# niessner/BundleFusion

Measured on AMD Instinct MI355X. Metric: frames/sec end-to-end (SIFT+SBA+TSDF re-integrate), 640x480 @4mm, higher is better.
Workload: dtype f32

## Files before the change

### bundlefusion_amd/csrc/solver.hip

```cpp
#include <hip/hip_runtime.h>

#include <algorithm>
#include <cstring>
#include <vector>

#include "bf_device.h"
#include "bf_resources.h"
#include "bf_se3.h"

using namespace bf;

namespace {

constexpr float FLOAT_EPSILON = 0.000001f;
constexpr uint32_t NOSLOT = 0xFFFFFFFFu;
constexpr int DENSE_BLK = 120;

typedef float f32x4 __attribute__((ext_vector_type(4)));

enum Flag { FL_DONE = 0, FL_NUM_SLOTS = 1, FL_NUM_PAIRS = 2, FL_LIST_LEN = 3, FL_GN_ITERS = 4, FL_BARRIER_FAIL = 5, FL_SLOT_OVERFLOW = 6, FL_PCG_ITERS = 8, FL_COUNT = 40 };

struct Cfg {
    float denseDistThresh, denseNormalThresh, denseColorThresh, denseColorGradientMin, denseDepthMin, denseDepthMax;
    uint32_t subsample;
    uint32_t W, H;
    float fx, fy, cx, cy;
    float wSparse, wDepth, wColor;
    int usePairwise;
};

struct Dev {
    const bf_entry_j* corr; uint32_t C;
    const int* valid; uint32_t N;
    float* xRot; float* xTrans;
    m44* T; m44* Tinv;
    uint32_t *keyCount, *keyStart, *cursor, *slotOfKey, *denseRaw, *keyPair;
    uint32_t *rowStart, *slotCol, *slotKey, *corrList;
    float *slotD, *slotO, *slotG, *slotP;
    float *diagA, *rhs, *prec;
    float *delta, *r, *p, *Ap;
    uint2* densePairs; float* denseWeight; float* denseBlocks;
    const bf_cached_frame* cache;
    int* flags;
    int* gridBar;
    float* energies;
    float* maxRes; int* maxIdx; int* highCount;
    int* numEntriesPerRow;
    float* coopVec;
    uint32_t* scanRow;
    float* maxResPart; int* maxIdxPart;
    uint32_t maxSlots, maxPairs;
};

BF_DEV f3 ld3(const float* p) { return mk3(p[0], p[1], p[2]); }
BF_DEV bool validCorr(const bf_entry_j& c) { return c.imgIdx_i != 0xFFFFFFFFu; }

__global__ void k_solve_begin(Dev d) {
    for (uint32_t k = threadIdx.x; k < (uint32_t)FL_COUNT; k += blockDim.x) d.flags[k] = 0;
    for (uint32_t k = threadIdx.x; k < 32u; k += blockDim.x) d.gridBar[k] = 0;
}

__global__ void k_poses(Dev d, uint32_t numKeys, int useDense) {
    const uint32_t i = blockIdx.x * blockDim.x + threadIdx.x;
    for (uint32_t k = i; k < numKeys; k += gridDim.x * blockDim.x) {
        d.keyCount[k] = 0u; d.cursor[k] = 0u;
        if (useDense) { d.denseRaw[k] = 0u; d.keyPair[k] = 0u; }
    }
    if (d.flags[FL_DONE]) return;
    if (i >= d.N) return;
    const m44 M = poseToMatrix(ld3(d.xRot + 3 * i), ld3(d.xTrans + 3 * i));
    d.T[i] = M;
    d.Tinv[i] = inverse44(M);
}

__global__ void k_key_count(Dev d) {
    if (d.flags[FL_DONE]) return;
    const uint32_t c = blockIdx.x * blockDim.x + threadIdx.x;
    if (c >= d.C) return;
    const bf_entry_j e = d.corr[c];
    if (!validCorr(e) || e.imgIdx_i >= d.N || e.imgIdx_j >= d.N) return;
    atomicAdd(&d.keyCount[e.imgIdx_i * d.N + e.imgIdx_j], 1u);
    atomicAdd(&d.keyCount[e.imgIdx_j * d.N + e.imgIdx_i], 1u);
}

__global__ void k_row_entries(Dev d) {
    const uint32_t i = blockIdx.x * blockDim.x + threadIdx.x;
    if (i >= d.N) return;
    uint32_t n = 0;
    for (uint32_t j = 0; j < d.N; ++j) n += d.keyCount[i * d.N + j];
    d.numEntriesPerRow[i] = (int)n;
}

BF_DEV void scanKey(const Dev& d, int useDense, uint32_t N, uint32_t i, uint32_t j, uint32_t& cnt, uint32_t& dn) {
    cnt = d.keyCount[i * N + j];
    dn = (useDense && i != j) ? d.denseRaw[min(i, j) * N + max(i, j)] : 0u;
}

__global__ __launch_bounds__(64) void k_scan_rows(Dev d, int useDense) {
    if (d.flags[FL_DONE]) return;
    const uint32_t N = d.N, i = blockIdx.x, lane = threadIdx.x;
    uint32_t a = 0, b = 0, c = 0;
    for (uint32_t j = lane; j < N; j += 64) {
        uint32_t cnt, dn;
        scanKey(d, useDense, N, i, j, cnt, dn);
        a += cnt; b += (cnt > 0 || dn) ? 1u : 0u; c += (dn && i < j) ? 1u : 0u;
    }
    a = (uint32_t)wave_sum_i((int)a); b = (uint32_t)wave_sum_i((int)b); c = (uint32_t)wave_sum_i((int)c);
    if (lane == 0) { d.scanRow[i * 3 + 0] = a; d.scanRow[i * 3 + 1] = b; d.scanRow[i * 3 + 2] = c; }
}

__global__ __launch_bounds__(1024) void k_scan_base(Dev d) {
    if (d.flags[FL_DONE]) return;
    __shared__ uint32_t sA[1024], sB[1024], sC[1024];
    const uint32_t N = d.N;
    const uint32_t chunk = (N + blockDim.x - 1) / blockDim.x;
    const uint32_t r0 = min(threadIdx.x * chunk, N), r1 = min(r0 + chunk, N);
    uint32_t a = 0, b = 0, c = 0;
    for (uint32_t r = r0; r < r1; ++r) { a += d.scanRow[r * 3]; b += d.scanRow[r * 3 + 1]; c += d.scanRow[r * 3 + 2]; }
    sA[threadIdx.x] = a; sB[threadIdx.x] = b; sC[threadIdx.x] = c;
    __syncthreads();
    for (uint32_t off = 1; off < blockDim.x; off <<= 1) {
        uint32_t ta = 0, tb = 0, tc = 0;
        if (threadIdx.x >= off) { ta = sA[threadIdx.x - off]; tb = sB[threadIdx.x - off]; tc = sC[threadIdx.x - off]; }
        __syncthreads();
// ... 266 lines not shown
                        if (tx >= 0 && ty >= 0 && tx < (int)c.W && ty < (int)c.H) {
                            float ci[4], ni[4];
                            bilinear<4>(u, v, tgt.d_cameraposDownsampled, c.W, c.H, ci);
                            if (ci[2] > c.denseDepthMin && ci[2] < c.denseDepthMax) {
                                bilinear<4>(u, v, tgt.d_normalsDownsampled, c.W, c.H, ni);
                                if (ni[0] != BF_MINF) {
                                    const f3 ct = mk3(ci[0], ci[1], ci[2]);
                                    const f3 nt = mk3(ni[0], ni[1], ni[2]);
                                    const float dist = len3(cst - ct);
                                    const float dN = n4[0] * ni[0] + n4[1] * ni[1] + n4[2] * ni[2] + n4[3] * ni[3];
                                    if (dN >= c.denseNormalThresh && dist <= c.denseDistThresh) {
                                        float jI[3][6], jJ[3][6];
                                        if (i > 0) derivI(TjI, Ti, cs, jI);
                                        if (j > 0) derivJ(TiI, Tj, cs, jJ);
                                        if (useDepth) {
                                            const f3 diff = ct - cst;
                                            Xd[12] = dot3(diff, nt);
                                            wd = c.wDepth * pw * powf(fmaxf(0.0f, 1.0f - ct.z / 2.0f), 2.5f);
#pragma unroll
                                            for (int k = 0; k < 6; ++k) {
                                                if (i > 0) Xd[k] = -(jI[0][k] * nt.x + jI[1][k] * nt.y + jI[2][k] * nt.z);
                                                if (j > 0) Xd[6 + k] = -(jJ[0][k] * nt.x + jJ[1][k] * nt.y + jJ[2][k] * nt.z);
                                            }
                                        }
                                        if (useColor) {
                                            float dI[2], iT;
                                            bilinear<2>(u, v, tgt.d_intensityDerivsDownsampled, c.W, c.H, dI);
                                            bilinear<1>(u, v, tgt.d_intensityDownsampled, c.W, c.H, &iT);
                                            const float res = iT - src.d_intensityDownsampled[idx];
                                            if (dI[0] != BF_MINF && fabsf(res) < c.denseColorThresh &&
                                                sqrtf(dI[0] * dI[0] + dI[1] * dI[1]) > c.denseColorGradientMin) {
                                                const float z2 = cst.z * cst.z;
                                                const float P00 = c.fx / cst.z, P02 = -c.fx * cst.x / z2, P11 = c.fy / cst.z, P12 = -c.fy * cst.y / z2;
                                                Xc[12] = res;
                                                wc = c.wColor * pw * fmaxf(0.0f, 1.0f - fabsf(res) / (1.15f * c.denseColorThresh));
#pragma unroll
                                                for (int k = 0; k < 6; ++k) {
                                                    if (i > 0) Xc[k] = dI[0] * (P00 * jI[0][k] + 0.0f * jI[1][k] + P02 * jI[2][k]) + dI[1] * (0.0f * jI[0][k] + P11 * jI[1][k] + P12 * jI[2][k]);
                                                    if (j > 0) Xc[6 + k] = dI[0] * (P00 * jJ[0][k] + 0.0f * jJ[1][k] + P02 * jJ[2][k]) + dI[1] * (0.0f * jJ[0][k] + P11 * jJ[1][k] + P12 * jJ[2][k]);
                                                }
                                            }
                                        }
                                    }
                                }
                            }
                        }
                    }
                }
            }
#pragma unroll
            for (int pass = 0; pass < 2; ++pass) {
                if (pass == 0 && !useDepth) continue;
                if (pass == 1 && !useColor) continue;
#pragma unroll
                for (int k = 0; k < 13; ++k) tileX[wave][lane][k] = pass == 0 ? Xd[k] : Xc[k];
                tileX[wave][lane][13] = 0.0f; tileX[wave][lane][14] = 0.0f; tileX[wave][lane][15] = 0.0f;
                tileW[wave][lane] = pass == 0 ? wd : wc;
                __syncthreads();
#pragma unroll
                for (int g = 0; g < 16; g += 2) {
                    const int r0 = 4 * g + (int)(lane >> 4), r1 = r0 + 4;
                    const float b0 = tileX[wave][r0][lane & 15], b1 = tileX[wave][r1][lane & 15];
                    acc0 = __builtin_amdgcn_mfma_f32_16x16x4f32(tileW[wave][r0] * b0, b0, acc0, 0, 0, 0);
                    acc1 = __builtin_amdgcn_mfma_f32_16x16x4f32(tileW[wave][r1] * b1, b1, acc1, 0, 0, 0);
                }
                __syncthreads();
            }
        }
#pragma unroll
        for (int r = 0; r < 4; ++r) part[wave][(4 * (lane >> 4) + r) * 16 + (lane & 15)] = acc0[r] + acc1[r];
        __syncthreads();
        if (threadIdx.x < DENSE_BLK) {
            const uint32_t t = threadIdx.x;
            uint32_t row, col;
            if (t < 36) { row = t / 6; col = t % 6; }
            else if (t < 72) { row = 6 + (t - 36) / 6; col = 6 + (t - 36) % 6; }
            else if (t < 108) { row = (t - 72) / 6; col = 6 + (t - 72) % 6; }
            else if (t < 114) { row = t - 108; col = 12; }
            else { row = 6 + (t - 114); col = 12; }
            const uint32_t e = row * 16 + col;
            out[t] = ((part[0][e] + part[1][e]) + part[2][e]) + part[3][e];
        }
        __syncthreads();
    }
}

__global__ __launch_bounds__(256) void k_slots(Dev d, Cfg c, int useDense) {
    if (d.flags[FL_DONE]) return;
    const uint32_t nSlots = (uint32_t)d.flags[FL_NUM_SLOTS];
    const uint32_t lane = threadIdx.x & 63;
    const uint32_t wavesPerGrid = gridDim.x * (blockDim.x >> 6);
    for (uint32_t s = blockIdx.x * (blockDim.x >> 6) + (threadIdx.x >> 6); s < nSlots; s += wavesPerGrid) {
        const uint32_t key = d.slotKey[s];
        const uint32_t start = d.keyStart[key], cnt = d.keyCount[key];
        const uint32_t a = lane / 6, b = lane % 6;
        float accD = 0.0f, accO = 0.0f;
        uint32_t prev = 0;
        bool first = true;
        for (uint32_t k = 0; k < cnt; ++k) {
            uint32_t best = 0xFFFFFFFFu;
            for (uint32_t t = lane; t < cnt; t += 64) {
                const uint32_t v = d.corrList[start + t];
                if ((first || v > prev) && v < best) best = v;
            }
#pragma unroll
            for (int o = 32; o > 0; o >>= 1) { const uint32_t t = __shfl_xor(best, o, 64); best = t < best ? t : best; }
            prev = best; first = false;
            const bf_entry_j e = d.corr[best >> 1];
            const bool roleB = best & 1u;
            const m44 TI = d.T[e.imgIdx_i], TJ = d.T[e.imgIdx_j];
            const f3 wi = xform(TI, mk3(e.pos_i[0], e.pos_i[1], e.pos_i[2]));
            const f3 wj = xform(TJ, mk3(e.pos_j[0], e.pos_j[1], e.pos_j[2]));
            const f3 r = wi - wj;
            const f3 wx = roleB ? wj : wi, wy = roleB ? wi : wj;
            const float sx = roleB ? -1.0f : 1.0f;
            auto col = [](f3 w, uint32_t q) -> f3 {
                switch (q) {
                    case 0: return mk3(1.0f, 0.0f, 0.0f);
                    case 1: return mk3(0.0f, 1.0f, 0.0f);
                    case 2: return mk3(0.0f, 0.0f, 1.0f);
                    case 3: return mk3(0.0f, -w.z, w.y);
                    case 4: return mk3(w.z, 0.0f, -w.x);
                    default: return mk3(-w.y, w.x, 0.0f);
                }
            };
            if (lane < 36) {
                const f3 ja = col(wx, a);
                accD += dot3(ja, col(wx, b));
                accO += -dot3(ja, col(wy, b));
            } else if (lane < 42) {
                accD += sx * dot3(col(wx, lane - 36), r);
            } else if (lane < 45) {
                const f3 jq = col(wx, lane - 42 + 3);
                accD += dot3(jq, jq);
            } else if (lane == 45) {
                accD += 1.0f;
            }
        }
        float dD = 0.0f, dO = 0.0f;
        if (useDense) {
            const uint32_t pp = d.keyPair[key];
            if (pp) {
                const float* blk = d.denseBlocks + (size_t)(pp - 1) * DENSE_BLK;
                const uint32_t i = key / d.N, j = key % d.N;
                const bool fwd = i < j;
                if (lane < 36) {
                    dD = fwd ? blk[a * 6 + b] : blk[36 + a * 6 + b];
                    dO = fwd ? blk[72 + a * 6 + b] : blk[72 + b * 6 + a];
                } else if (lane < 42) {
                    dD = fwd ? blk[108 + (lane - 36)] : blk[114 + (lane - 36)];
                }
            }
        }
        if (lane < 36) {
            d.slotD[(size_t)s * 36 + lane] = c.wSparse * accD + dD;
            d.slotO[(size_t)s * 36 + lane] = c.wSparse * accO + dO;
        } else if (lane < 42) {
            d.slotG[(size_t)s * 6 + (lane - 36)] = c.wSparse * accD + dD;
        } else if (lane < 46) {
            d.slotP[(size_t)s * 4 + (lane - 42)] = accD;
        }
    }
}

__global__ __launch_bounds__(256) void k_rows(Dev d) {
    if (d.flags[FL_DONE]) return;
// ... 498 lines not shown
}

__global__ __launch_bounds__(64) void k_max_residual_final(Dev d, uint32_t G) {
    float best = 0.0f; int bi = 0;
    if (threadIdx.x < G) { best = d.maxResPart[threadIdx.x]; bi = d.maxIdxPart[threadIdx.x]; }
#pragma unroll
    for (int o = 32; o > 0; o >>= 1) {
        const float ov = __shfl_xor(best, o, 64); const int oi = __shfl_xor(bi, o, 64);
        if (maxResBetter(ov, oi, best, bi)) { best = ov; bi = oi; }
    }
    if (threadIdx.x == 0) { d.maxRes[0] = best; d.maxIdx[0] = bi; }
}

__global__ void k_count_high(Dev d, float w, float thresh) {
    const uint32_t c = blockIdx.x * blockDim.x + threadIdx.x;
    bool hi = false;
    if (c < d.C) hi = absMaxResidual(d, d.corr[c], w) > thresh;
    const unsigned long long m = __ballot(hi);
    if ((threadIdx.x & 63) == 0 && m) atomicAdd(d.highCount, __popcll(m));
}

__global__ __launch_bounds__(1024) void k_energy(Dev d, float w, uint32_t slot, int honourDone) {
    if (honourDone && d.flags[FL_DONE] && slot > (uint32_t)d.flags[FL_GN_ITERS]) return;
    __shared__ float sh[16];
    float part = 0.0f;
    for (uint32_t c = threadIdx.x; c < d.C; c += blockDim.x) {
        const bf_entry_j e = d.corr[c];
        if (!validCorr(e)) continue;
        const m44 TI = poseToMatrix(ld3(d.xRot + 3 * e.imgIdx_i), ld3(d.xTrans + 3 * e.imgIdx_i));
        const m44 TJ = poseToMatrix(ld3(d.xRot + 3 * e.imgIdx_j), ld3(d.xTrans + 3 * e.imgIdx_j));
        const f3 r = xform(TI, mk3(e.pos_i[0], e.pos_i[1], e.pos_i[2])) - xform(TJ, mk3(e.pos_j[0], e.pos_j[1], e.pos_j[2]));
        part += w * dot3(r, r);
    }
    const float tot = blockSum(part, sh);
    if (threadIdx.x == 0) d.energies[slot] = tot;
}

__global__ void k_matrices_to_poses(const m44* T, uint32_t n, float* rot3, float* trans3, const int* valid) {
    const uint32_t i = blockIdx.x * blockDim.x + threadIdx.x;
    if (i < n && valid[i]) {
        f3 r, t;
        matrixToPose(T[i], r, t);
        rot3[3 * i] = r.x; rot3[3 * i + 1] = r.y; rot3[3 * i + 2] = r.z;
        trans3[3 * i] = t.x; trans3[3 * i + 1] = t.y; trans3[3 * i + 2] = t.z;
    }
}
__global__ void k_poses_to_matrices(const float* rot3, const float* trans3, uint32_t n, m44* T, const int* valid) {
    const uint32_t i = blockIdx.x * blockDim.x + threadIdx.x;
    if (i < n && valid[i]) T[i] = poseToMatrix(ld3(rot3 + 3 * i), ld3(trans3 + 3 * i));
}

__global__ void k_expand_dense(Dev d, float* JtJ, float* Jtr) {
    const uint32_t nPairs = (uint32_t)d.flags[FL_NUM_PAIRS];
    const uint32_t dim = 6 * d.N;
    for (uint32_t p = 0; p < nPairs; ++p) {
        const uint2 pr = d.densePairs[p];
        const float* blk = d.denseBlocks + (size_t)p * DENSE_BLK;
        const uint32_t t = threadIdx.x;
        if (t < 36) {
            const uint32_t a = t / 6, b = t % 6;
            JtJ[(size_t)(pr.x * 6 + a) * dim + pr.x * 6 + b] += blk[a * 6 + b];
            JtJ[(size_t)(pr.y * 6 + a) * dim + pr.y * 6 + b] += blk[36 + a * 6 + b];
            JtJ[(size_t)(pr.x * 6 + a) * dim + pr.y * 6 + b] += blk[72 + a * 6 + b];
            JtJ[(size_t)(pr.y * 6 + b) * dim + pr.x * 6 + a] += blk[72 + a * 6 + b];
        } else if (t < 42) {
            Jtr[pr.x * 6 + (t - 36)] += blk[108 + (t - 36)];
            Jtr[pr.y * 6 + (t - 36)] += blk[114 + (t - 36)];
        }
        __syncthreads();
    }
}

}

struct bf_solver {
    bf_solver_config cfg;
    uint32_t maxImages, maxResiduals, maxCorrPerImage;
    Dev d{};
    hipStream_t stream = nullptr;
    bf::Resources res;
    std::vector<float> convergence;
    float hMaxRes = 0.0f; int hMaxIdx = 0; int hBarrierFail = 0;
    bool pcgWide = true;
    int pcgGroups = -1;
    uint32_t maxCoopGroups = COOP_MAX_GROUPS;
    bool forceVecGlobal = false;
    size_t coopVecFloats = 0;
    uint32_t lastN = 0, lastGNrequested = 0;
    float lastWeightSparse = 1.0f;
    bool lastUsedDense = false;
};

extern "C" {

int bf_solver_create(uint32_t maxNumberOfImages, uint32_t maxNumResiduals, const bf_solver_config* cfg, bf_solver** out) {
    BF_REQUIRE(cfg && out, "null argument");
    BF_REQUIRE(maxNumberOfImages >= 2 && maxNumResiduals > 0, "bad capacity");
    bf_solver* s = new bf_solver();
    bf::CreateGuard<bf_solver> guard(s, bf_solver_destroy);
    s->cfg = *cfg;
    s->maxImages = maxNumberOfImages; s->maxResiduals = maxNumResiduals;
    BF_HIP_TRY(hipFuncSetAttribute(reinterpret_cast<const void*>(&k_pcg<true>), hipFuncAttributeMaxDynamicSharedMemorySize, (int)PCG_LDS_MAX));
    BF_HIP_TRY(hipFuncSetAttribute(reinterpret_cast<const void*>(&k_pcg_coop<COOP_THREADS>), hipFuncAttributeMaxDynamicSharedMemorySize, (int)PCG_LDS_MAX));
    BF_HIP_TRY(hipFuncSetAttribute(reinterpret_cast<const void*>(&k_pcg_small<1>), hipFuncAttributeMaxDynamicSharedMemorySize, (int)PCG_LDS_MAX));
    BF_HIP_TRY(hipFuncSetAttribute(reinterpret_cast<const void*>(&k_pcg_small<2>), hipFuncAttributeMaxDynamicSharedMemorySize, (int)PCG_LDS_MAX));
    BF_HIP_TRY(hipFuncSetAttribute(reinterpret_cast<const void*>(&k_pcg_small<3>), hipFuncAttributeMaxDynamicSharedMemorySize, (int)PCG_LDS_MAX));
    BF_HIP_TRY(hipFuncSetAttribute(reinterpret_cast<const void*>(&k_pcg_small<4>), hipFuncAttributeMaxDynamicSharedMemorySize, (int)PCG_LDS_MAX));
    if (const char* e = getenv("BF_PCG_WIDE")) s->pcgWide = atoi(e) != 0;
    if (const char* e = getenv("BF_PCG_GROUPS")) s->pcgGroups = atoi(e);
    if (const char* e = getenv("BF_PCG_VEC_GLOBAL")) s->forceVecGlobal = atoi(e) != 0;
    {
        int dev = 0, cus = 0;
        if (hipGetDevice(&dev) == hipSuccess && hipDeviceGetAttribute(&cus, hipDeviceAttributeMultiprocessorCount, dev) == hipSuccess && cus > 0)
            s->maxCoopGroups = std::max(1u, std::min(COOP_MAX_GROUPS, (uint32_t)cus / 2u));
        else (void)hipGetLastError();
    }
    s->maxCorrPerImage = std::min(std::max(maxNumResiduals / maxNumberOfImages, 1000u), 4000u);
    const size_t N = maxNumberOfImages, M = N * N, C = maxNumResiduals;
    Dev& d = s->d;
    d.maxSlots = (uint32_t)std::min<size_t>(M, 2 * C + (N <= 64 ? M : 4 * N));
    d.maxPairs = (uint32_t)(N * (N - 1) / 2);
    if (N > 64) d.maxPairs = (uint32_t)std::min<size_t>(d.maxPairs, d.maxSlots);
    s->coopVecFloats = ((31 * N + 4096 <= PCG_LDS_MAX / 4 && !s->forceVecGlobal) ? (size_t)4 : (size_t)s->maxCoopGroups * ((31 * N + 1 + 3) & ~(size_t)3));
    bf::Resources& R = s->res;
    BF_TRY(R.device(&d.T, N)); BF_TRY(R.device(&d.Tinv, N)); BF_TRY(R.device(&d.keyCount, M)); BF_TRY(R.device(&d.keyStart, M)); BF_TRY(R.device(&d.cursor, M));
    BF_TRY(R.device(&d.slotOfKey, M)); BF_TRY(R.device(&d.denseRaw, M)); BF_TRY(R.device(&d.keyPair, M)); BF_TRY(R.device(&d.rowStart, N + 1));
    BF_TRY(R.device(&d.slotCol, (size_t)d.maxSlots)); BF_TRY(R.device(&d.slotKey, (size_t)d.maxSlots)); BF_TRY(R.device(&d.corrList, 2 * C));
    BF_TRY(R.device(&d.slotD, (size_t)d.maxSlots * 36)); BF_TRY(R.device(&d.slotO, (size_t)d.maxSlots * 36)); BF_TRY(R.device(&d.slotG, (size_t)d.maxSlots * 6));
    BF_TRY(R.device(&d.slotP, (size_t)d.maxSlots * 4)); BF_TRY(R.device(&d.diagA, N * 36)); BF_TRY(R.device(&d.rhs, N * 6)); BF_TRY(R.device(&d.prec, N * 6));
    BF_TRY(R.device(&d.delta, N * 6)); BF_TRY(R.device(&d.r, N * 6)); BF_TRY(R.device(&d.p, N * 6)); BF_TRY(R.device(&d.Ap, N * 6));
    BF_TRY(R.device(&d.densePairs, (size_t)d.maxPairs)); BF_TRY(R.device(&d.denseWeight, (size_t)d.maxPairs));
    BF_TRY(R.device(&d.denseBlocks, (size_t)d.maxPairs * DENSE_BLK)); BF_TRY(R.device(&d.flags, FL_COUNT)); BF_TRY(R.device(&d.gridBar, 32)); BF_TRY(R.device(&d.energies, 40));
    BF_TRY(R.device(&d.maxRes, 1)); BF_TRY(R.device(&d.maxIdx, 1)); BF_TRY(R.device(&d.highCount, 1)); BF_TRY(R.device(&d.numEntriesPerRow, N));
    BF_TRY(R.device(&d.scanRow, 3 * (N + 1))); BF_TRY(R.device(&d.coopVec, s->coopVecFloats)); BF_TRY(R.device(&d.maxResPart, MAXRES_GROUPS)); BF_TRY(R.device(&d.maxIdxPart, MAXRES_GROUPS));
    (void)hipMemset(d.flags, 0, FL_COUNT * sizeof(int));
    *out = guard.dismiss();
    return BF_OK;
}

int bf_solver_destroy(bf_solver* s) {
    if (!s) return BF_OK;
    (void)hipStreamSynchronize(s->stream);
    delete s;
    return BF_OK;
}

int bf_solver_set_stream(bf_solver* s, void* st) { BF_REQUIRE(s, "null solver"); s->stream = (hipStream_t)st; return BF_OK; }

int bf_solver_solve(bf_solver* s, bf_entry_j* d_corr, uint32_t numCorr, const int32_t* d_valid, uint32_t N, uint32_t nNonLin, uint32_t nLin,
                    const bf_cached_frame* d_cache, uint32_t cw, uint32_t ch, const float K4[4], const float* wS, const float* wDD,
                    const float* wDC, uint32_t numWeights, int usePairwise, float* d_rot, float* d_trans, int rebuildJT, int findMaxResidual,
                    uint32_t revalidateIdx) {
    (void)rebuildJT; (void)revalidateIdx;
    BF_REQUIRE(s && d_valid && d_rot && d_trans && wS && wDD && wDC, "null argument");
    BF_REQUIRE(numCorr == 0 || d_corr, "null correspondences");
    nNonLin = std::min(nNonLin, numWeights);
    BF_REQUIRE(N > 1 && nNonLin > 0 && nLin > 0, "numberOfImages > 1 && nNonLinearIterations > 0 required");
    BF_REQUIRE(N <= s->maxImages && numCorr <= s->maxResiduals, "problem exceeds the solver's capacity");
    BF_REQUIRE(nNonLin <= 32, "at most 32 non-linear iterations");
    Dev d = s->d;
    d.corr = d_corr; d.C = numCorr; d.valid = d_valid; d.N = N; d.xRot = d_rot; d.xTrans = d_trans; d.cache = d_cache;
    s->d = d;
    Cfg c;
    c.denseDistThresh = s->cfg.denseDistThresh; c.denseNormalThresh = s->cfg.denseNormalThresh; c.denseColorThresh = s->cfg.denseColorThresh;
    c.denseColorGradientMin = s->cfg.denseColorGradientMin; c.denseDepthMin = s->cfg.denseDepthMin; c.denseDepthMax = s->cfg.denseDepthMax;
    c.subsample = s->cfg.denseOverlapCheckSubsampleFactor;
    c.W = cw; c.H = ch;
    if (d_cache) {
        BF_REQUIRE(K4, "cache intrinsics missing");
        BF_REQUIRE(c.subsample > 0 && cw / c.subsample > 8, "denseDepthWidth / subsample factor must exceed 8");
        BF_REQUIRE((cw / c.subsample) * (ch / c.subsample) <= 512, "overlap pre-filter samples exceed one workgroup");
        c.fx = K4[0]; c.fy = K4[1]; c.cx = K4[2]; c.cy = K4[3];
    } else { c.fx = c.fy = c.cx = c.cy = 0.0f; }
    c.usePairwise = usePairwise;
    hipStream_t st = s->stream;
    const size_t M = (size_t)N * N;
    hipLaunchKernelGGL(k_solve_begin, dim3(1), dim3(64), 0, st, d);
    const bool record = s->cfg.recordConvergence != 0;
    if (record) hipLaunchKernelGGL(k_energy, dim3(1), dim3(1024), 0, st, d, wS[0], 0u, 0);
    bool anyDense = false, prevDense = false;
    for (uint32_t it = 0; it < nNonLin; ++it) {
        c.wSparse = wS[it]; c.wDepth = wDD[it]; c.wColor = wDC[it];
        const int useDense = (d_cache != nullptr) && (c.wDepth > 0.0f || c.wColor > 0.0f);
        anyDense |= useDense != 0;
        const bool reuse = it > 0 && !useDense && !prevDense;
        prevDense = useDense != 0;
        hipLaunchKernelGGL(k_poses, dim3(std::max<uint32_t>(div_up(N, 256), std::min<uint32_t>(div_up((uint32_t)M, 256), 128u))), dim3(256), 0, st, d, reuse ? 0u : (uint32_t)M, useDense);
        if (useDense) {
            const dim3 grid = usePairwise ? dim3(N, N) : dim3(N - 1, 1);
            hipLaunchKernelGGL(k_dense_overlap, grid, dim3(512), 0, st, d, c);
        }
        if (!reuse) {
            if (numCorr) hipLaunchKernelGGL(k_key_count, dim3(div_up(numCorr, 256)), dim3(256), 0, st, d);
            if (it == 0) hipLaunchKernelGGL(k_row_entries, dim3(div_up(N, 64)), dim3(64), 0, st, d);
            hipLaunchKernelGGL(k_scan_rows, dim3(N), dim3(64), 0, st, d, useDense);
            hipLaunchKernelGGL(k_scan_base, dim3(1), dim3(1024), 0, st, d);
            hipLaunchKernelGGL(k_scan_fill, dim3(N), dim3(64), 0, st, d, useDense);
            if (numCorr) hipLaunchKernelGGL(k_fill, dim3(div_up(numCorr, 256)), dim3(256), 0, st, d);
        }
        if (useDense) {
            const uint32_t g = std::min<uint32_t>(std::max<uint32_t>(N * (N - 1) / 2, 1u), 1024u);
            hipLaunchKernelGGL(k_dense_weight, dim3(g), dim3(256), 0, st, d, c);
            hipLaunchKernelGGL(k_dense_build, dim3(g), dim3(256), 0, st, d, c);
        }
        hipLaunchKernelGGL(k_slots, dim3(std::min<uint32_t>(div_up(d.maxSlots, 4), 2048u)), dim3(256), 0, st, d, c, useDense);
        hipLaunchKernelGGL(k_rows, dim3(div_up(N, 4)), dim3(256), 0, st, d);
        {
            uint32_t G = N <= 32 ? 1u : std::min(s->maxCoopGroups, div_up(N - 1, COOP_ROWS_PER_GROUP));
            if (s->pcgGroups > 0) G = std::min(std::min<uint32_t>((uint32_t)s->pcgGroups, N - 1), s->maxCoopGroups);
            const uint32_t rpg = div_up(N - 1, G);
            size_t baseFloats = ((size_t)31 * N + 1 + (size_t)rpg * 36 + 3) & ~(size_t)3;
            const uint32_t vecGlobal = (s->forceVecGlobal || baseFloats + 37 * 8 > PCG_LDS_MAX / 4) ? 1u : 0u;
            if (vecGlobal) baseFloats = ((size_t)rpg * 36 + 3) & ~(size_t)3;
            const size_t ldsFloats = std::min<size_t>(PCG_LDS_MAX / 4, baseFloats + (size_t)rpg * std::min<uint32_t>(N - 1, 96u) * 37);
            const bool vecFits = !vecGlobal || (size_t)G * (((size_t)31 * N + 1 + 3) & ~(size_t)3) <= s->coopVecFloats;
            if (s->pcgGroups != 0 && nNonLin <= 32 && vecFits && baseFloats + 37 * 8 <= PCG_LDS_MAX / 4)
            {
                if (s->pcgWide && G == 1 && 6 * N <= COOP_THREADS && !vecGlobal) {
                    const uint32_t waves = std::min(SMALL_MAX_WAVES, std::max(8u, 4u * div_up(div_up(N - 1, SMALL_TRIPS), 4u)));
                    const size_t smallBase = (size_t)(waves + 2) * SMALL_VEC;
                    const uint32_t smallLds = (uint32_t)std::min<size_t>(PCG_LDS_MAX / 4, smallBase + std::max<size_t>(8, (size_t)(N - 1) * (N - 1) * 37));
                    const dim3 block(waves * 64);
                    const int lastGN = (int)(it == nNonLin - 1);
                    switch (div_up(6 * N - 6, 64)) {
                        case 1: hipLaunchKernelGGL(k_pcg_small<1>, dim3(1), block, smallLds * 4, st, d, nLin, it, lastGN, smallLds); break;
                        case 2: hipLaunchKernelGGL(k_pcg_small<2>, dim3(1), block, smallLds * 4, st, d, nLin, it, lastGN, smallLds); break;
                        case 3: hipLaunchKernelGGL(k_pcg_small<3>, dim3(1), block, smallLds * 4, st, d, nLin, it, lastGN, smallLds); break;
                        default: hipLaunchKernelGGL(k_pcg_small<4>, dim3(1), block, smallLds * 4, st, d, nLin, it, lastGN, smallLds); break;
                    }
                }
                else
                    hipLaunchKernelGGL(k_pcg_coop<COOP_THREADS>, dim3(G), dim3(COOP_THREADS), ldsFloats * 4, st, d, nLin, it, (int)(it == nNonLin - 1), (uint32_t)ldsFloats, vecGlobal);
            }
            else if ((size_t)N * 124 + 4 <= PCG_LDS_MAX)
                hipLaunchKernelGGL(k_pcg<true>, dim3(1), dim3(1024), (size_t)N * 124 + 4, st, d, nLin, it, (int)(it == nNonLin - 1));
            else hipLaunchKernelGGL(k_pcg<false>, dim3(1), dim3(1024), 0, st, d, nLin, it, (int)(it == nNonLin - 1));
        }
        if (record) hipLaunchKernelGGL(k_energy, dim3(1), dim3(1024), 0, st, d, c.wSparse, it + 1, 1);
    }
    BF_HIP_TRY(hipGetLastError());
    s->lastN = N; s->lastGNrequested = nNonLin; s->lastWeightSparse = wS[nNonLin - 1]; s->lastUsedDense = anyDense;
    if (findMaxResidual) {
        if (s->lastWeightSparse > 0.0f && numCorr > 0) {
            const uint32_t gmr = std::min<uint32_t>(MAXRES_GROUPS, std::max<uint32_t>(1u, div_up(numCorr, 1024u)));
            hipLaunchKernelGGL(k_max_residual, dim3(gmr), dim3(1024), 0, st, d, s->lastWeightSparse);
            hipLaunchKernelGGL(k_max_residual_final, dim3(1), dim3(64), 0, st, d, gmr);
            BF_HIP_TRY(hipMemcpyAsync(&s->hMaxRes, d.maxRes, 4, hipMemcpyDeviceToHost, st));
            BF_HIP_TRY(hipMemcpyAsync(&s->hMaxIdx, d.maxIdx, 4, hipMemcpyDeviceToHost, st));
            BF_HIP_TRY(hipMemcpyAsync(&s->hBarrierFail, d.flags + FL_BARRIER_FAIL, 4, hipMemcpyDeviceToHost, st));
            BF_HIP_TRY(hipStreamSynchronize(st));
            BF_REQUIRE(s->hBarrierFail == 0, "PCG grid barrier timed out (a workgroup of k_pcg_coop was never scheduled)");
        } else { s->hMaxRes = 0.0f; s->hMaxIdx = 0; }
    }
    if (record) {
        int flags[FL_COUNT];
        float en[40];
        BF_HIP_TRY(hipMemcpyAsync(flags, d.flags, sizeof flags, hipMemcpyDeviceToHost, st));
        BF_HIP_TRY(hipMemcpyAsync(en, d.energies, sizeof en, hipMemcpyDeviceToHost, st));
        BF_HIP_TRY(hipStreamSynchronize(st));
        s->convergence.assign(nNonLin + 1, -1.0f);
        for (int k = 0; k <= flags[FL_GN_ITERS] && k <= (int)nNonLin; ++k) s->convergence[k] = en[k];
    }
    return BF_OK;
}

int bf_solver_get_var_to_corr_num_entries_per_row(bf_solver* s, const int32_t** d_out) {
    BF_REQUIRE(s && d_out, "null argument");
    *d_out = s->d.numEntriesPerRow;
    return BF_OK;
}

int bf_solver_get_corr_overflow(bf_solver* s, uint32_t* numImagesOverLimit, uint32_t* limit) {
    BF_REQUIRE(s && numImagesOverLimit, "null argument");
    if (limit) *limit = s->maxCorrPerImage;
    *numImagesOverLimit = 0;
    const uint32_t N = s->lastN;
    if (N == 0) return BF_OK;
    std::vector<int> rows(N);
    BF_HIP_TRY(hipMemcpyAsync(rows.data(), s->d.numEntriesPerRow, sizeof(int) * N, hipMemcpyDeviceToHost, s->stream));
    BF_HIP_TRY(hipStreamSynchronize(s->stream));
    for (int r : rows) if ((uint32_t)std::max(r, 0) > s->maxCorrPerImage) (*numImagesOverLimit)++;
    return BF_OK;
}

int bf_solver_get_max_residual(bf_solver* s, float* mx, int32_t* idx) {
    BF_REQUIRE(s && mx && idx, "null argument");
// ... 121 lines not shown
```

Baseline: 1566.

## Fuse dense weight and build into a four-way split kernel with ticket reduction

Adds k_dense_wide, which replaces the separate k_dense_weight and k_dense_build launches by a single kernel that assigns four blocks per image pair. Each block recounts overlap to get the pair weight, builds Jacobian rows for a quarter of the pixels, and accumulates the Gram matrix with MFMA. The quarters are combined through a partial buffer plus an atomic ticket, so the last block to arrive reduces them. The goal is more parallelism per pair and one fewer launch, at the cost of every block redundantly recomputing the overlap count and of cross-block fence and atomic synchronisation.

```diff
diff --git a/bundlefusion_amd/csrc/solver.hip b/bundlefusion_amd/csrc/solver.hip
--- a/bundlefusion_amd/csrc/solver.hip
+++ b/bundlefusion_amd/csrc/solver.hip
@@ -40,6 +40,7 @@
     float *diagA, *rhs, *prec;
     float *delta, *r, *p, *Ap;
     uint2* densePairs; float* denseWeight; float* denseBlocks;
+    float* densePart; uint32_t* denseTicket;
     const bf_cached_frame* cache;
     int* flags;
     int* gridBar;
@@ -472,6 +473,298 @@
             out[t] = ((part[0][e] + part[1][e]) + part[2][e]) + part[3][e];
         }
         __syncthreads();
+    }
+}
+
+constexpr uint32_t DW_WAVES = 4, DW_THREADS = DW_WAVES * 64, DW_COLS = 13, DW_PIX = 10;
+constexpr uint32_t DW_MAX_PAIRS = 2048;
+
+struct DenseWideLds {
+    float X[DW_WAVES][2][64][DW_COLS];
+    float W[DW_WAVES][2][64];
+    float acc[2][4][64];
+    float m[4][3][3];
+    float trI[16];
+    int wcount[DW_WAVES];
+    uint32_t last;
+};
+
+BF_DEV void derivIUniform(const m44& A, const m44& D, float m[4][3][3], float trI[16]) {
+    const m44 tr = mul44(A, D);
+#pragma unroll
+    for (int e = 0; e < 16; ++e) trI[e] = tr.e[e];
+#pragma unroll
+    for (int k = 0; k < 4; ++k) {
+        const float vx = D.e[k], vy = D.e[4 + k], vz = D.e[8 + k];
+        const float sk[3][3] = {{0.0f, -vz, vy}, {vz, 0.0f, -vx}, {-vy, vx, 0.0f}};
+#pragma unroll
+        for (int r = 0; r < 3; ++r)
+#pragma unroll
+            for (int cc = 0; cc < 3; ++cc)
+                m[k][r][cc] = (A.e[r * 4 + 0] * sk[0][cc] + A.e[r * 4 + 1] * sk[1][cc] + A.e[r * 4 + 2] * sk[2][cc]) * -1.0f;
+    }
+}
+BF_DEV void derivIShared(const m44& A, const float (*m)[3][3], const float* trI, f3 p, float jac[3][6]) {
+    const float pt[3] = {p.x - trI[3], p.y - trI[7], p.z - trI[11]};
+#pragma unroll
+    for (int r = 0; r < 3; ++r) {
+#pragma unroll
+        for (int cc = 0; cc < 3; ++cc) {
+            jac[r][cc] = (-trI[0 * 4 + r]) * A.e[0 * 4 + cc] + (-trI[1 * 4 + r]) * A.e[1 * 4 + cc] + (-trI[2 * 4 + r]) * A.e[2 * 4 + cc];
+            float acc = pt[0] * m[r][0][cc];
+            acc += pt[1] * m[r][1][cc];
+            acc += pt[2] * m[r][2][cc];
+            acc += (-trI[0 * 4 + r]) * m[3][0][cc];
+            acc += (-trI[1 * 4 + r]) * m[3][1][cc];
+            acc += (-trI[2 * 4 + r]) * m[3][2][cc];
+            jac[r][3 + cc] = acc;
+        }
+    }
+}
+
+template <int K> struct Taps { float v[4][K]; bool in[4]; };
+template <int K>
+BF_DEV void loadTaps(float x, float y, const float* __restrict__ in, uint32_t W, uint32_t H, Taps<K>& t) {
+    const int x0 = (int)floorf(x), y0 = (int)floorf(y);
+#pragma unroll
+    for (int q = 0; q < 4; ++q) {
+        const int px = x0 + (q & 1), py = y0 + (q >> 1);
+        t.in[q] = (uint32_t)px < W && (uint32_t)py < H;
+        const float* v = in + (t.in[q] ? (size_t)K * ((size_t)py * W + px) : (size_t)0);
+        if (K == 4) { const float4 f = *reinterpret_cast<const float4*>(v); t.v[q][0] = f.x; t.v[q][1 % K] = f.y; t.v[q][2 % K] = f.z; t.v[q][3 % K] = f.w; }
+        else if (K == 2) { const float2 f = *reinterpret_cast<const float2*>(v); t.v[q][0] = f.x; t.v[q][1 % K] = f.y; }
+        else t.v[q][0] = v[0];
+    }
+}
+template <int K>
+BF_DEV bool combineTaps(float x, float y, const Taps<K>& t, float* out) {
+    const int x0 = (int)floorf(x), y0 = (int)floorf(y);
+    const float alpha = x - (float)x0, beta = y - (float)y0;
+    float s0[K], s1[K], w0 = 0.0f, w1 = 0.0f;
+#pragma unroll
+    for (int k = 0; k < K; ++k) { s0[k] = 0.0f; s1[k] = 0.0f; }
+#define BF_TAP(Q, WGT, S, WS) \
+    if (t.in[Q] && t.v[Q][0] != BF_MINF) { _Pragma("unroll") for (int k = 0; k < K; ++k) S[k] += (WGT) * t.v[Q][k]; WS += (WGT); }
+    BF_TAP(0, 1.0f - alpha, s0, w0)
+    BF_TAP(1, alpha, s0, w0)
+    BF_TAP(2, 1.0f - alpha, s1, w1)
+    BF_TAP(3, alpha, s1, w1)
+#undef BF_TAP
+    float ss[K], ww = 0.0f;
+#pragma unroll
+    for (int k = 0; k < K; ++k) ss[k] = 0.0f;
+    if (w0 > 0.0f) { _Pragma("unroll") for (int k = 0; k < K; ++k) ss[k] += (1.0f - beta) * (s0[k] / w0); ww += (1.0f - beta); }
+    if (w1 > 0.0f) { _Pragma("unroll") for (int k = 0; k < K; ++k) ss[k] += beta * (s1[k] / w1); ww += beta; }
+    if (ww > 0.0f) { _Pragma("unroll") for (int k = 0; k < K; ++k) out[k] = ss[k] / ww; return true; }
+#pragma unroll
+    for (int k = 0; k < K; ++k) out[k] = BF_MINF;
+    return false;
+}
+
+BF_DEV void denseRows(const Cfg& c, const bf_cached_frame& tgt, const bf_cached_frame& src, const float (*mI)[3][3], const float* trI, const m44& Tj, const m44& TiI, const m44& TjI,
+                      const m44& tr, uint32_t i, uint32_t j, float pw, bool useDepth, bool useColor, uint32_t idx, uint32_t npix,
+                      float Xd[13], float Xc[13], float& wd, float& wc) {
+    wd = 0.0f; wc = 0.0f;
+#pragma unroll
+    for (int k = 0; k < 13; ++k) { Xd[k] = 0.0f; Xc[k] = 0.0f; }
+    const uint32_t ic = min(idx, npix - 1u);
+    const float4 cp4 = reinterpret_cast<const float4*>(src.d_cameraposDownsampled)[ic];
+    const float4 nj = reinterpret_cast<const float4*>(src.d_normalsDownsampled)[ic];
+    const float srcI = src.d_intensityDownsampled[ic];
+    bool ok = idx < npix && (cp4.z > c.denseDepthMin && cp4.z < c.denseDepthMax) && nj.x != BF_MINF;
+    const f3 cs = mk3(cp4.x, cp4.y, cp4.z);
+    const float n4[4] = {tr.e[0] * nj.x + tr.e[1] * nj.y + tr.e[2] * nj.z + tr.e[3] * nj.w,
+                         tr.e[4] * nj.x + tr.e[5] * nj.y + tr.e[6] * nj.z + tr.e[7] * nj.w,
+                         tr.e[8] * nj.x + tr.e[9] * nj.y + tr.e[10] * nj.z + tr.e[11] * nj.w,
+                         tr.e[12] * nj.x + tr.e[13] * nj.y + tr.e[14] * nj.z + tr.e[15] * nj.w};
+    const f3 cst = xform(tr, cs);
+    float u, v;
+    cameraToDepth(c, cst, u, v);
+    const int tx = f2i(roundf(u)), ty = f2i(roundf(v));
+    ok = ok && (tx >= 0 && ty >= 0 && tx < (int)c.W && ty < (int)c.H);
+    if (!ok) { u = 0.0f; v = 0.0f; }
+    Taps<4> tc, tn; Taps<2> td; Taps<1> ti;
+    loadTaps<4>(u, v, tgt.d_cameraposDownsampled, c.W, c.H, tc);
+    loadTaps<4>(u, v, tgt.d_normalsDownsampled, c.W, c.H, tn);
+    if (useColor) {
+        loadTaps<2>(u, v, tgt.d_intensityDerivsDownsampled, c.W, c.H, td);
+        loadTaps<1>(u, v, tgt.d_intensityDownsampled, c.W, c.H, ti);
+    }
+    if (!ok) return;
+    float ci[4], ni[4];
+    combineTaps<4>(u, v, tc, ci);
+    if (!(ci[2] > c.denseDepthMin && ci[2] < c.denseDepthMax)) return;
+    combineTaps<4>(u, v, tn, ni);
+    if (!(ni[0] != BF_MINF)) return;
+    const f3 ct = mk3(ci[0], ci[1], ci[2]);
+    const f3 nt = mk3(ni[0], ni[1], ni[2]);
+    const float dist = len3(cst - ct);
+    const float dN = n4[0] * ni[0] + n4[1] * ni[1] + n4[2] * ni[2] + n4[3] * ni[3];
+    if (!(dN >= c.denseNormalThresh && dist <= c.denseDistThresh)) return;
+    float jI[3][6], jJ[3][6];
+    if (i > 0) derivIShared(TjI, mI, trI, cs, jI);
+    if (j > 0) derivJ(TiI, Tj, cs, jJ);
+    if (useDepth) {
+        const f3 diff = ct - cst;
+        Xd[12] = dot3(diff, nt);
+        wd = c.wDepth * pw * powf(fmaxf(0.0f, 1.0f - ct.z / 2.0f), 2.5f);
+#pragma unroll
+        for (int k = 0; k < 6; ++k) {
+            if (i > 0) Xd[k] = -(jI[0][k] * nt.x + jI[1][k] * nt.y + jI[2][k] * nt.z);
+            if (j > 0) Xd[6 + k] = -(jJ[0][k] * nt.x + jJ[1][k] * nt.y + jJ[2][k] * nt.z);
+        }
+    }
+    if (useColor) {
+        float dI[2], iT;
+        combineTaps<2>(u, v, td, dI);
+        combineTaps<1>(u, v, ti, &iT);
+        const float res = iT - srcI;
+        if (dI[0] != BF_MINF && fabsf(res) < c.denseColorThresh && sqrtf(dI[0] * dI[0] + dI[1] * dI[1]) > c.denseColorGradientMin) {
+            const float z2 = cst.z * cst.z;
+            const float P00 = c.fx / cst.z, P02 = -c.fx * cst.x / z2, P11 = c.fy / cst.z, P12 = -c.fy * cst.y / z2;
+            Xc[12] = res;
+            wc = c.wColor * pw * fmaxf(0.0f, 1.0f - fabsf(res) / (1.15f * c.denseColorThresh));
+#pragma unroll
+            for (int k = 0; k < 6; ++k) {
+                if (i > 0) Xc[k] = dI[0] * (P00 * jI[0][k] + 0.0f * jI[1][k] + P02 * jI[2][k]) + dI[1] * (0.0f * jI[0][k] + P11 * jI[1][k] + P12 * jI[2][k]);
+                if (j > 0) Xc[6 + k] = dI[0] * (P00 * jJ[0][k] + 0.0f * jJ[1][k] + P02 * jJ[2][k]) + dI[1] * (0.0f * jJ[0][k] + P11 * jJ[1][k] + P12 * jJ[2][k]);
+            }
+        }
+    }
+}
+
+__global__ __launch_bounds__(DW_THREADS, 2) void k_dense_wide(Dev d, Cfg c) {
+    if (d.flags[FL_DONE]) return;
+    __shared__ DenseWideLds S;
+    const uint32_t nPairs = min((uint32_t)d.flags[FL_NUM_PAIRS], DW_MAX_PAIRS);
+    const uint32_t npix = c.W * c.H;
+    const uint32_t tid = threadIdx.x, wave = tid >> 6, lane = tid & 63;
+    const uint32_t nTrips = (npix + 255u) / 256u;
+    const bool useDepth = c.wDepth > 0.0f, useColor = c.wColor > 0.0f;
+    for (uint32_t q = blockIdx.x; q < 4u * nPairs; q += gridDim.x) {
+        const uint32_t p = q >> 2, w = q & 3u;
+        const uint2 pr = d.densePairs[p];
+        const uint32_t i = pr.x, j = pr.y;
+        const m44 Ti = d.T[i], Tj = d.T[j], TiI = d.Tinv[i], TjI = d.Tinv[j];
+        const m44 tr = mul44(TiI, Tj);
+        const bf_cached_frame tgt = d.cache[i], src = d.cache[j];
+        if (tid == 0u && i > 0u) derivIUniform(TjI, Ti, S.m, S.trI);
+        int count = 0;
+        for (uint32_t base = 0; base < npix; base += DW_THREADS * DW_PIX) {
+            float dep[DW_PIX]; uchar4 nu[DW_PIX];
+#pragma unroll
+            for (uint32_t k = 0; k < DW_PIX; ++k) {
+                const uint32_t idx = min(base + k * DW_THREADS + tid, npix - 1u);
+                dep[k] = src.d_depthDownsampled[idx];
+                nu[k] = reinterpret_cast<const uchar4*>(src.d_normalsDownsampledUCHAR4)[idx];
+            }
+            f3 nj[DW_PIX], qq[DW_PIX]; bool ok[DW_PIX]; float dt[DW_PIX]; uchar4 nt[DW_PIX]; int tx[DW_PIX], ty[DW_PIX];
+#pragma unroll
+            for (uint32_t k = 0; k < DW_PIX; ++k) {
+                const uint32_t idx = base + k * DW_THREADS + tid, ic = min(idx, npix - 1u);
+                const uint32_t x = ic % c.W, y = ic / c.W;
+                const f3 cp = depthToCamera(c, (int)x, (int)y, dep[k]);
+                ok[k] = idx < npix && (cp.z > c.denseDepthMin && cp.z < c.denseDepthMax) && (nu[k].x | nu[k].y | nu[k].z | nu[k].w);
+                nj[k] = mk3((float)nu[k].x / 255.0f * 2.0f - 1.0f, (float)nu[k].y / 255.0f * 2.0f - 1.0f, (float)nu[k].z / 255.0f * 2.0f - 1.0f);
+                nj[k] = rot(tr, nj[k]);
+                qq[k] = xform(tr, cp);
+                float u, v;
+                cameraToDepth(c, qq[k], u, v);
+                tx[k] = f2i(roundf(u)); ty[k] = f2i(roundf(v));
+                ok[k] = ok[k] && (tx[k] >= 0 && ty[k] >= 0 && tx[k] < (int)c.W && ty[k] < (int)c.H);
+                const uint32_t ti = ok[k] ? (uint32_t)(ty[k] * (int)c.W + tx[k]) : 0u;
+                dt[k] = tgt.d_depthDownsampled[ti];
+                nt[k] = reinterpret_cast<const uchar4*>(tgt.d_normalsDownsampledUCHAR4)[ti];
+            }
+#pragma unroll
+            for (uint32_t k = 0; k < DW_PIX; ++k) {
+                const f3 ct = depthToCamera(c, tx[k], ty[k], dt[k]);
+                const f3 nT = mk3((float)nt[k].x / 255.0f * 2.0f - 1.0f, (float)nt[k].y / 255.0f * 2.0f - 1.0f, (float)nt[k].z / 255.0f * 2.0f - 1.0f);
+                if (ok[k] && (ct.z > c.denseDepthMin && ct.z < c.denseDepthMax) && (nt[k].x | nt[k].y | nt[k].z | nt[k].w) &&
+                    dot3(nj[k], nT) >= c.denseNormalThresh && len3(qq[k] - ct) <= c.denseDistThresh) count++;
+            }
+        }
+        count = wave_sum_i(count);
+        __syncthreads();
+        if (lane == 0) S.wcount[wave] = count;
+        __syncthreads();
+        int total = 0;
+#pragma unroll
+        for (uint32_t k = 0; k < DW_WAVES; ++k) total += S.wcount[k];
+        float pw = (float)total;
+        if (pw > 0) { if (pw < 800) pw = 0; else pw = 1.0f / fminf(logf(pw), 9.0f); }
+        if (w == 0u && tid == 0u) d.denseWeight[p] = pw;
+        float* out = d.denseBlocks + (size_t)p * DENSE_BLK;
+        if (pw == 0.0f) {
+            if (w == 0u && tid < DENSE_BLK) out[tid] = 0.0f;
+            continue;
+        }
+        f32x4 acc = {0.0f, 0.0f, 0.0f, 0.0f};
+        for (uint32_t t0 = 0; t0 < nTrips; t0 += DW_WAVES) {
+            if (t0 + wave < nTrips) {
+                float Xd[13], Xc[13], wd, wc;
+                denseRows(c, tgt, src, S.m, S.trI, Tj, TiI, TjI, tr, i, j, pw, useDepth, useColor, 256u * (t0 + wave) + 64u * w + lane, npix, Xd, Xc, wd, wc);
+#pragma unroll
+                for (int k = 0; k < 13; ++k) { S.X[wave][0][lane][k] = Xd[k]; S.X[wave][1][lane][k] = Xc[k]; }
+                S.W[wave][0][lane] = wd; S.W[wave][1][lane] = wc;
+            }
+            __syncthreads();
+            if (wave < 2u) {
+                const uint32_t nt = min(DW_WAVES, nTrips - t0), col = lane & 15u;
+                for (uint32_t t = 0; t < nt; ++t) {
+#pragma unroll
+                    for (int pass = 0; pass < 2; ++pass) {
+                        if (pass == 0 && !useDepth) continue;
+                        if (pass == 1 && !useColor) continue;
+#pragma unroll
+                        for (uint32_t g = 0; g < 16; g += 2) {
+                            const uint32_t row = 4u * (g + wave) + (lane >> 4);
+                            const float x = S.X[t][pass][row][min(col, DW_COLS - 1u)];
+                            const float b = col < DW_COLS ? x : 0.0f;
+                            acc = __builtin_amdgcn_mfma_f32_16x16x4f32(S.W[t][pass][row] * b, b, acc, 0, 0, 0);
+                        }
+                    }
+                }
+            }
+            __syncthreads();
+        }
+        if (wave < 2u) {
+#pragma unroll
+            for (int r = 0; r < 4; ++r) S.acc[wave][r][lane] = acc[r];
+        }
+        __syncthreads();
+        float* part = d.densePart + (size_t)p * 1024u;
+        static_assert(DW_THREADS == 256, "one thread per element of the chain's 16 x 16 Gram");
+        {
+            const uint32_t r = wave;
+            part[w * 256u + (4u * (lane >> 4) + r) * 16u + (lane & 15u)] = S.acc[0][r][lane] + S.acc[1][r][lane];
+        }
+        asm volatile("s_waitcnt vmcnt(0)" ::: "memory");
+        __syncthreads();
+        if (tid == 0u) {
+            __builtin_amdgcn_fence(__ATOMIC_RELEASE, "agent");
+            asm volatile("s_waitcnt vmcnt(0)" ::: "memory");
+            const uint32_t ticket = __hip_atomic_fetch_add(&d.denseTicket[p], 1u, __ATOMIC_RELAXED, __HIP_MEMORY_SCOPE_AGENT);
+            S.last = ticket == 3u ? 1u : 0u;
+            if (S.last) {
+                __builtin_amdgcn_fence(__ATOMIC_ACQUIRE, "agent");
+                d.denseTicket[p] = 0u;
+                asm volatile("s_waitcnt vmcnt(0)" ::: "memory");
+            }
+        }
+        __syncthreads();
+        if (!S.last) continue;
+        if (tid < DENSE_BLK) {
+            const uint32_t t = tid;
+            uint32_t row, col;
+            if (t < 36) { row = t / 6; col = t % 6; }
+            else if (t < 72) { row = 6 + (t - 36) / 6; col = 6 + (t - 36) % 6; }
+            else if (t < 108) { row = (t - 72) / 6; col = 6 + (t - 72) % 6; }
+            else if (t < 114) { row = t - 108; col = 12; }
+            else { row = 6 + (t - 114); col = 12; }
+            const uint32_t e = row * 16 + col;
+            out[t] = ((part[e] + part[256u + e]) + part[512u + e]) + part[768u + e];
+        }
     }
 }
 
@@ -1136,6 +1429,7 @@
     std::vector<float> convergence;
     float hMaxRes = 0.0f; int hMaxIdx = 0; int hBarrierFail = 0;
     bool pcgWide = true;
+    bool denseWide = true;
     int pcgGroups = -1;
     uint32_t maxCoopGroups = COOP_MAX_GROUPS;
     bool forceVecGlobal = false;
@@ -1161,6 +1455,7 @@
     BF_HIP_TRY(hipFuncSetAttribute(reinterpret_cast<const void*>(&k_pcg_small<3>), hipFuncAttributeMaxDynamicSharedMemorySize, (int)PCG_LDS_MAX));
     BF_HIP_TRY(hipFuncSetAttribute(reinterpret_cast<const void*>(&k_pcg_small<4>), hipFuncAttributeMaxDynamicSharedMemorySize, (int)PCG_LDS_MAX));
     if (const char* e = getenv("BF_PCG_WIDE")) s->pcgWide = atoi(e) != 0;
+    if (const char* e = getenv("BF_DENSE_WIDE")) s->denseWide = atoi(e) != 0;
     if (const char* e = getenv("BF_PCG_GROUPS")) s->pcgGroups = atoi(e);
     if (const char* e = getenv("BF_PCG_VEC_GLOBAL")) s->forceVecGlobal = atoi(e) != 0;
     {
@@ -1184,10 +1479,13 @@
     BF_TRY(R.device(&d.slotP, (size_t)d.maxSlots * 4)); BF_TRY(R.device(&d.diagA, N * 36)); BF_TRY(R.device(&d.rhs, N * 6)); BF_TRY(R.device(&d.prec, N * 6));
     BF_TRY(R.device(&d.delta, N * 6)); BF_TRY(R.device(&d.r, N * 6)); BF_TRY(R.device(&d.p, N * 6)); BF_TRY(R.device(&d.Ap, N * 6));
     BF_TRY(R.device(&d.densePairs, (size_t)d.maxPairs)); BF_TRY(R.device(&d.denseWeight, (size_t)d.maxPairs));
+    const size_t widePairs = std::min<size_t>(d.maxPairs, DW_MAX_PAIRS);
+    BF_TRY(R.device(&d.densePart, widePairs * 1024)); BF_TRY(R.device(&d.denseTicket, widePairs));
     BF_TRY(R.device(&d.denseBlocks, (size_t)d.maxPairs * DENSE_BLK)); BF_TRY(R.device(&d.flags, FL_COUNT)); BF_TRY(R.device(&d.gridBar, 32)); BF_TRY(R.device(&d.energies, 40));
     BF_TRY(R.device(&d.maxRes, 1)); BF_TRY(R.device(&d.maxIdx, 1)); BF_TRY(R.device(&d.highCount, 1)); BF_TRY(R.device(&d.numEntriesPerRow, N));
     BF_TRY(R.device(&d.scanRow, 3 * (N + 1))); BF_TRY(R.device(&d.coopVec, s->coopVecFloats)); BF_TRY(R.device(&d.maxResPart, MAXRES_GROUPS)); BF_TRY(R.device(&d.maxIdxPart, MAXRES_GROUPS));
     (void)hipMemset(d.flags, 0, FL_COUNT * sizeof(int));
+    (void)hipMemset(d.denseTicket, 0, widePairs * sizeof(uint32_t));
     *out = guard.dismiss();
     return BF_OK;
 }
@@ -1254,8 +1552,13 @@
         }
         if (useDense) {
             const uint32_t g = std::min<uint32_t>(std::max<uint32_t>(N * (N - 1) / 2, 1u), 1024u);
-            hipLaunchKernelGGL(k_dense_weight, dim3(g), dim3(256), 0, st, d, c);
-            hipLaunchKernelGGL(k_dense_build, dim3(g), dim3(256), 0, st, d, c);
+            const uint32_t pairsAtMost = std::min<uint32_t>(usePairwise ? N * (N - 1) / 2 : N - 1, d.maxPairs);
+            if (s->denseWide && pairsAtMost <= DW_MAX_PAIRS)
+                hipLaunchKernelGGL(k_dense_wide, dim3(4 * g), dim3(DW_THREADS), 0, st, d, c);
+            else {
+                hipLaunchKernelGGL(k_dense_weight, dim3(g), dim3(256), 0, st, d, c);
+                hipLaunchKernelGGL(k_dense_build, dim3(g), dim3(256), 0, st, d, c);
+            }
         }
         hipLaunchKernelGGL(k_slots, dim3(std::min<uint32_t>(div_up(d.maxSlots, 4), 2048u)), dim3(256), 0, st, d, c, useDense);
         hipLaunchKernelGGL(k_rows, dim3(div_up(N, 4)), dim3(256), 0, st, d);
```

After: 1590 (median of 6 runs). +1.5%, better.
